# KyungMinJin/OTPose

Measured on AMD Instinct MI355X. Metric: frames/sec at 384x288, 5-frame window, batch 16; heatmap max-abs delta vs ref, higher is better.
Workload: dtype f32 storage+accumulate / f16x3 split products; 1 GPU; BASELINE configs[1]: batch 16 x 5-frame x 384x288, HRNet-W48 + DCN warp + ConvVideoTransformer, fp32 forward (eval), seeded synthetic weights; clips_per_gpu=16, parallelism=dp1, outputs_finite=True

## Files before the change

### include/otpose_hip.h

```cpp
#ifndef OTPOSE_HIP_H
#define OTPOSE_HIP_H

#include <stddef.h>

#ifdef __cplusplus
extern "C" {
#endif

#define OTP_OK 0
#define OTP_ERR_BAD_ARG (-1)
#define OTP_ERR_UNSUPPORTED (-2)
#define OTP_ERR_LAUNCH (-3)
#define OTP_ERR_WORKSPACE (-4)

#define OTP_DTYPE_F32 0
#define OTP_DTYPE_F16 1
#define OTP_DTYPE_BF16 2
#define OTP_DTYPE_F64 3
#define OTP_DTYPE_I64 4

#define OTP_ACT_NONE 0
#define OTP_ACT_RELU 1
#define OTP_ACT_GELU 2

// ... 188 lines not shown
int otp_mlp_fused(const void* x, const void* packed, const void* scale, const void* shift, const void* res, void* out,
                  int B, int C, int HID, int T, void* stream);
int otp_ln_mlp_fused(const void* y, const void* ln_gamma, const void* ln_beta, float ln_eps, const void* packed,
                     const void* scale, const void* shift, void* out, int B, int C, int HID, int T, void* stream);

int otp_dense_x3_supported(int C, int T);
size_t otp_dense_x3_weight_bytes(int C);
int otp_dense_x3_pack(const void* w, const void* scale, const void* shift, void* packed, int C, void* stream);
int otp_dense_x3(const void* const* x, const void* const* packed, const void* const* res, void* const* out, int nprob, int B,
                 int C, int T, void* stream);
int otp_dense_x3_pack_bf16p(const void* w, const void* scale, const void* shift, void* packed, int C, void* stream);
int otp_dense_x3_bf16p(const void* const* x, const void* const* packed, const void* const* res, void* const* out, int nprob, int B,
                 int C, int T, void* stream);
int otp_qkv_front_x3(const void* x, const void* table, const void* packed_q, const void* packed_k, const void* packed_v,
                     void* q, void* k, void* v, int B, int C, int T, float eps, void* stream);

int otp_stem_conv_x3_supported(int B, int F, int H, int W, int Cout);
size_t otp_stem_conv_x3_weight_bytes(int Cout);
int otp_stem_conv_x3_pack(const void* w, const void* scale, const void* shift, void* packed, int Cout, void* stream);
int otp_stem_conv_x3(const void* in, const void* packed, void* out, int B, int F, int H, int W, int Cout, void* stream);

int otp_pointwise_x3_supported(int Cin, int Cout, int T);
size_t otp_pointwise_x3_weight_bytes(int Cin, int Cout);
int otp_pointwise_x3_pack(const void* w, const void* scale, const void* shift, void* packed, int Cin, int Cout, void* stream);
int otp_pointwise_x3(const void* x, const void* packed, const void* res, void* out, int B, int Cin, int Cout, int T, int x_ctot,
                     int x_coff, int res_ctot, int res_coff, int out_ctot, int out_coff, int relu, void* stream);
int otp_pointwise_x3_s8_supported(int Cin, int Cout, int T);
size_t otp_pointwise_x3_s8_weight_bytes(int Cin, int Cout);
int otp_pointwise_x3_s8_pack(const void* w, const void* scale, const void* shift, void* packed, int Cin, int Cout, void* stream);
int otp_pointwise_x3_s8(const void* x, const void* packed, void* out_s8, int B, int Cin, int Cout, int T, int x_ctot, int x_coff,
// ... 219 lines not shown
```

### otpose_amd/csrc/densex.hip

```cpp
#include "x3.h"
#ifndef OTP_ENTRY
#define OTP_ENTRY(name) name
#endif

namespace {

constexpr int dx_ks(int C) { return (C + 31) / 32; }
constexpr int dx_block_bytes(int C) { return (dx_ks(C) * 2 * 1024 + 128 + 4095) / 4096 * 4096; }

__global__ void densex_pack_kernel(const float* __restrict__ w, const float* __restrict__ scale, const float* __restrict__ shift,
                                   unsigned char* __restrict__ packed, int C) {
    const int KS = dx_ks(C), MT = (C + 15) / 16, BLKB = dx_block_bytes(C), units = BLKB / 16;
    const int idx = blockIdx.x * blockDim.x + threadIdx.x;
    if (idx >= MT * units) return;
    const int mt = idx / units, u = idx - mt * units;
    otp_u32x4 o = {0u, 0u, 0u, 0u};
    if (u < KS * 2 * 64) {
        const int frag = u >> 6, lane = u & 63, row = 16 * mt + (lane & 15), kq = lane >> 4, ks = frag >> 1;
        float v[8];
#pragma unroll
        for (int j = 0; j < 8; ++j) {
            const int c = 32 * ks + 8 * kq + j;
            v[j] = (row < C && c < C) ? w[(size_t)row * C + c] : 0.f;
        }
// ... 2 lines not shown
        o = __builtin_bit_cast(otp_u32x4, (frag & 1) ? lo : hi);
    } else if (u < KS * 2 * 64 + 8) {
        const int k = (u - KS * 2 * 64) * 4;
        float v[4];
#pragma unroll
        for (int i = 0; i < 4; ++i) {
            const int e = k + i, c = 16 * mt + (e & 15);
            v[i] = c < C ? (e < 16 ? (scale ? scale[c] : 1.f) : (shift ? shift[c] : 0.f)) : 0.f;
        }
        o = (otp_u32x4){__builtin_bit_cast(uint32_t, v[0]), __builtin_bit_cast(uint32_t, v[1]), __builtin_bit_cast(uint32_t, v[2]),
                    __builtin_bit_cast(uint32_t, v[3])};
    }
    reinterpret_cast<otp_u32x4*>(packed)[idx] = o;
}

template <int C, bool RES, bool H1 = false>
__device__ __forceinline__ void dx_project(const otp_x3x8 (&Xh)[dx_ks(C)][2], const otp_x3x8 (&Xl)[dx_ks(C)][2],
                                           const unsigned char* __restrict__ packed, unsigned char* lds,
                                           const float* __restrict__ res, float* __restrict__ out, size_t base, int T, int tok,
                                           bool valid, unsigned* rflag) {
    constexpr int KS = dx_ks(C), MT = (C + 15) / 16, BLKB = dx_block_bytes(C);
    bool bad = false;
    const int lane = threadIdx.x & 63, kq = lane >> 4;
    const unsigned plane = (unsigned)((size_t)C * T * sizeof(float));
    const otp_rsrc ro = make_rsrc32(out + base, plane);
    const otp_rsrc rr = make_rsrc32(RES && res ? res + base : out, RES && res ? plane : 0u);
#pragma unroll 1
    for (int mt = 0; mt < MT; ++mt) {
        int voff[4];
        otp_f32x2 r[4];
#pragma unroll
        for (int i = 0; i < 4; ++i) {
            const int c = 16 * mt + 4 * kq + i;
            voff[i] = (valid && c < C) ? (c * T + tok) * 4 : -16;
            if (RES) r[i] = __builtin_bit_cast(otp_f32x2, __builtin_amdgcn_raw_buffer_load_b64(rr, voff[i], 0, 0));
        }
        asm volatile("" ::: "memory");
        if (mt + 1 < MT) otp_lds_stage<256, BLKB>(packed + (size_t)(mt + 1) * BLKB, lds + ((mt + 1) & 1) * BLKB);
        asm volatile("" ::: "memory");
        const unsigned char* P = lds + (mt & 1) * BLKB;
        otp_f32x4 acc0 = {0.f, 0.f, 0.f, 0.f}, acc1 = {0.f, 0.f, 0.f, 0.f};
#pragma unroll
        for (int ks = 0; ks < KS; ++ks) {
            const otp_x3x8 ah = *reinterpret_cast<const otp_x3x8*>(P + (ks * 2) * 1024 + lane * 16);
            if constexpr (!H1) {
                const otp_x3x8 al = *reinterpret_cast<const otp_x3x8*>(P + (ks * 2 + 1) * 1024 + lane * 16);
                acc0 = OTP_X3_MFMA(al, Xh[ks][0], acc0, 0, 0, 0);
                acc1 = OTP_X3_MFMA(al, Xh[ks][1], acc1, 0, 0, 0);
                acc0 = OTP_X3_MFMA(ah, Xl[ks][0], acc0, 0, 0, 0);
                acc1 = OTP_X3_MFMA(ah, Xl[ks][1], acc1, 0, 0, 0);
            }
            acc0 = OTP_X3_MFMA(ah, Xh[ks][0], acc0, 0, 0, 0);
            acc1 = OTP_X3_MFMA(ah, Xh[ks][1], acc1, 0, 0, 0);
        }
        const otp_f32x4 sc = *reinterpret_cast<const otp_f32x4*>(P + KS * 2048 + 16 * kq);
        const otp_f32x4 sh = *reinterpret_cast<const otp_f32x4*>(P + KS * 2048 + 64 + 16 * kq);
#pragma unroll
        for (int i = 0; i < 4; ++i) {
            otp_f32x2 v = {acc0[i] * sc[i] + sh[i], acc1[i] * sc[i] + sh[i]};
            if (RES) v += r[i];
            bad |= otp_out_of_range(v.x);
                bad |= otp_out_of_range(v.y);
            __builtin_amdgcn_raw_buffer_store_b64(__builtin_bit_cast(otp_u32x2, v), ro, voff[i], 0, 0);
        }
        if (mt + 1 < MT) {
            asm volatile("s_waitcnt vmcnt(4)" ::: "memory");
            __builtin_amdgcn_s_barrier();
            asm volatile("" ::: "memory");
        }
    }
    otp_range_report(rflag, bad, OTP_RANGE_DENSEX);
}

struct DxArgs {
    const float* x[3];
    const unsigned char* packed[3];
    const float* res[3];
    float* out[3];
};

template <int C, bool H1 = false>
// ... 19 lines not shown
            v0[j] = live ? v.x : 0.f;
            v1[j] = live ? v.y : 0.f;
        }
        otp_x3_split8(v0, Xh[ks][0], Xl[ks][0]);
        otp_x3_split8(v1, Xh[ks][1], Xl[ks][1]);
    }
    __syncthreads();
    dx_project<C, true, H1>(Xh, Xl, A.packed[blockIdx.y], lds, A.res[blockIdx.y], A.out[blockIdx.y], base, T, tok, valid, rflag);
}

struct QxArgs {
    const unsigned char* packed[3];
    float* out[3];
};

template <int C, bool H1 = false>
__global__ __launch_bounds__(256, C <= 136 ? 3 : 1) void qkvx_front_kernel(const float* __restrict__ x, const float* __restrict__ table,
                                                            QxArgs A, int T, int tiles_per_b, float eps, unsigned* rflag) {
    constexpr int KS = dx_ks(C), BLKB = dx_block_bytes(C), TAB = 3 * C * 8;
    __shared__ __attribute__((aligned(16))) unsigned char lds[2 * BLKB];
    __shared__ __attribute__((aligned(16))) float tab[TAB];
    const int tid = threadIdx.x, lane = tid & 63, wave = tid >> 6, kq = lane >> 4, n = lane & 15;
    const int b = blockIdx.x / tiles_per_b, tile = blockIdx.x - b * tiles_per_b;
    const int tok = tile * 128 + wave * 32 + 2 * n;
    const bool valid = tok < T;
    const int tokc = valid ? tok : T - 2;
    const bool l_ok = tokc >= 1, r_ok = tokc + 2 < T;
    const size_t base = (size_t)b * C * T;
    const otp_rsrc rx = make_rsrc(x + base, (size_t)C * T * sizeof(float));
    constexpr float inv_c = 1.f / (float)C;
    const int vb0 = (8 * kq * T + tokc) * 4;
    for (int i = tid; i < TAB / 4; i += 256)
        reinterpret_cast<otp_f32x4*>(tab)[i] = reinterpret_cast<const otp_f32x4*>(table)[i];
    __syncthreads();

    for (int p = (int)blockIdx.y; p <= (int)blockIdx.y; ++p) {
        otp_lds_stage<256, BLKB>(A.packed[p], lds);
        const float* tp = tab + p * C * 8;
        float X0[KS][8], X1[KS][8];
        float s0 = 0.f, s1 = 0.f;
#pragma unroll
        for (int ks = 0; ks < KS; ++ks) {
#pragma unroll
            for (int j = 0; j < 8; ++j) {
                const int c = 32 * ks + 8 * kq + j;
                const bool live = 32 * ks + 24 + j < C || c < C;
                const int so = (32 * ks + j) * T * 4;
                const otp_f32x2 m = __builtin_bit_cast(otp_f32x2, __builtin_amdgcn_raw_buffer_load_b64(rx, live ? vb0 : -16, so, 0));
                const float la = bload(rx, live ? vb0 - 4 : -16, so), ld = bload(rx, live ? vb0 + 8 : -16, so);
                const float a = l_ok ? la : 0.f, d = r_ok ? ld : 0.f;
                const otp_f32x4 w = *reinterpret_cast<const otp_f32x4*>(tp + (live ? c : 0) * 8);
                X0[ks][j] = live ? w[0] * a + w[1] * m.x + w[2] * m.y : 0.f;
// ... 18 lines not shown
        otp_x3x8 Xh[KS][2], Xl[KS][2];
#pragma unroll
        for (int ks = 0; ks < KS; ++ks) {
#pragma unroll
            for (int j = 0; j < 8; ++j) {
                const int c = 32 * ks + 8 * kq + j;
                const bool live = 32 * ks + 24 + j < C || c < C;
                const float g = tp[(live ? c : 0) * 8 + 3], be = tp[(live ? c : 0) * 8 + 4];
                X0[ks][j] = live ? X0[ks][j] * r0 * g + be : 0.f;
                X1[ks][j] = live ? X1[ks][j] * r1 * g + be : 0.f;
            }
            otp_x3_split8(X0[ks], Xh[ks][0], Xl[ks][0]);
            otp_x3_split8(X1[ks], Xh[ks][1], Xl[ks][1]);
        }
        __syncthreads();
        dx_project<C, false, H1>(Xh, Xl, A.packed[p], lds, nullptr, A.out[p], base, T, tok, valid, rflag);
    }
}

}

#ifndef OTP_X3_GRAD_COPY
extern "C" int otp_dense_x3_supported(int C, int T) { return ((C == 136 || C == 204) && T > 0 && T % 2 == 0) ? 1 : 0; }

extern "C" size_t otp_dense_x3_weight_bytes(int C) {
    if (C <= 0 || C % 4) return 0;
    return (size_t)((C + 15) / 16) * dx_block_bytes(C);
}
#endif

extern "C" int OTP_ENTRY(otp_dense_x3_pack)(const void* w, const void* scale, const void* shift, void* packed, int C, void* stream) {
// ... 41 lines not shown
                            int nprob, int B, int C, int T, void* stream) {
    return dx_dense_launch(x, packed, res, out, nprob, B, C, T, stream, false);
}

#ifndef OTP_X3_GRAD_COPY
extern "C" int otp_dense_h1(const void* const* x, const void* const* packed, const void* const* res, void* const* out, int nprob, int B,
                            int C, int T, void* stream) {
    return dx_dense_launch(x, packed, res, out, nprob, B, C, T, stream, true);
}
#endif

#ifndef OTP_X3_GRAD_COPY
namespace {
int dx_qkv_launch(const void* x, const void* table, const void* packed_q, const void* packed_k, const void* packed_v, void* q, void* k,
                  void* v, int B, int C, int T, float eps, void* stream, bool h1) {
    if (!x || !table || !packed_q || !packed_k || !packed_v || !q || !k || !v || B <= 0) return OTP_ERR_BAD_ARG;
    if (!otp_dense_x3_supported(C, T)) return OTP_ERR_UNSUPPORTED;
    if ((reinterpret_cast<uintptr_t>(x) | reinterpret_cast<uintptr_t>(q) | reinterpret_cast<uintptr_t>(k) |
         reinterpret_cast<uintptr_t>(v)) & 7 ||
        (reinterpret_cast<uintptr_t>(table) | reinterpret_cast<uintptr_t>(packed_q) | reinterpret_cast<uintptr_t>(packed_k) |
         reinterpret_cast<uintptr_t>(packed_v)) & 15)
        return OTP_ERR_BAD_ARG;
    if ((size_t)C * T * sizeof(float) >= (1ull << 31)) return OTP_ERR_UNSUPPORTED;
    QxArgs a;
    a.packed[0] = static_cast<const unsigned char*>(packed_q); a.packed[1] = static_cast<const unsigned char*>(packed_k);
    a.packed[2] = static_cast<const unsigned char*>(packed_v);
    a.out[0] = static_cast<float*>(q); a.out[1] = static_cast<float*>(k); a.out[2] = static_cast<float*>(v);
    const int tiles = otp_ceil_div(T, 128);
    const dim3 grid((unsigned)(B * tiles), 3u);
    auto st = static_cast<hipStream_t>(stream);
    auto xf = static_cast<const float*>(x), tf = static_cast<const float*>(table);
    if (C == 204) {
        if (h1) hipLaunchKernelGGL((qkvx_front_kernel<204, true>), grid, dim3(256), 0, st, xf, tf, a, T, tiles, eps, otp_range_word());
        else hipLaunchKernelGGL((qkvx_front_kernel<204, false>), grid, dim3(256), 0, st, xf, tf, a, T, tiles, eps, otp_range_word());
    } else {
        if (h1) hipLaunchKernelGGL((qkvx_front_kernel<136, true>), grid, dim3(256), 0, st, xf, tf, a, T, tiles, eps, otp_range_word());
        else hipLaunchKernelGGL((qkvx_front_kernel<136, false>), grid, dim3(256), 0, st, xf, tf, a, T, tiles, eps, otp_range_word());
    }
    return otp_launch_status();
}
}

extern "C" int otp_qkv_front_x3(const void* x, const void* table, const void* packed_q, const void* packed_k,
                                const void* packed_v, void* q, void* k, void* v, int B, int C, int T, float eps, void* stream) {
    return dx_qkv_launch(x, table, packed_q, packed_k, packed_v, q, k, v, B, C, T, eps, stream, false);
}

extern "C" int otp_qkv_front_h1(const void* x, const void* table, const void* packed_q, const void* packed_k,
                                const void* packed_v, void* q, void* k, void* v, int B, int C, int T, float eps, void* stream) {
    return dx_qkv_launch(x, table, packed_q, packed_k, packed_v, q, k, v, B, C, T, eps, stream, true);
}
#endif
```

### otpose_amd/csrc/transformer.hip

```cpp
#include "common.h"
#include <cstdlib>
#ifndef OTP_ENTRY
#define OTP_ENTRY(name) name
#endif

namespace {

template <int CREG>
__global__ __launch_bounds__(256) void ln_channel_kernel(const float* __restrict__ x, const float* __restrict__ gamma,
                                                          const float* __restrict__ beta, float* __restrict__ y,
                                                          int C, int T, float eps) {
    const int t = blockIdx.x * blockDim.x + threadIdx.x;
    if (t >= T) return;
    const size_t base = (size_t)blockIdx.y * C * T + t;
    const float inv_c = 1.f / (float)C;
    if (CREG > 0) {
        float v[CREG > 0 ? CREG : 1];
        float s = 0.f;
#pragma unroll
        for (int c = 0; c < CREG; ++c) {
            v[c] = c < C ? x[base + (size_t)c * T] : 0.f;
            s += v[c];
        }
        const float mu = s * inv_c;
// ... 367 lines not shown
            }
        }
    }
    float* slab = slabs + ((size_t)bh * gridDim.y + s) * HSP * HSP;
#pragma unroll
    for (int i = 0; i < TPW; ++i) {
        const int tile = wave + 4 * i;
        if (tile < NT) {
            const int ib = tile / NB, jb = tile - ib * NB;
#pragma unroll
            for (int r = 0; r < 4; ++r) slab[(ib * 16 + kk * 4 + r) * HSP + jb * 16 + r16] = acc[i][r];
        }
    }
}

__global__ __launch_bounds__(256) void attn_softmax_kernel(const float* __restrict__ slabs, float* __restrict__ P,
                                                            int hs, int HSP, int NS, float scale) {
    const int bh = blockIdx.x, lane = threadIdx.x & 63, wave = threadIdx.x >> 6;
    const int row = blockIdx.y * 4 + wave;
    if (row >= HSP) return;
    const float* sb = slabs + (size_t)bh * NS * HSP * HSP;
    float* pb = P + (size_t)bh * HSP * HSP;
    float v[2];
#pragma unroll
    for (int h = 0; h < 2; ++h) {
        const int col = lane + 64 * h;
        const bool live = row < hs && col < hs;
        const float* sp = sb + (live ? (size_t)row * HSP + col : 0);
        float a = 0.f;
        int s = 0;
        for (; s + 8 <= NS; s += 8) {
            float t[8];
#pragma unroll
            for (int j = 0; j < 8; ++j) t[j] = sp[(size_t)(s + j) * HSP * HSP];
#pragma unroll
            for (int j = 0; j < 8; ++j) a += t[j];
        }
        for (; s < NS; ++s) a += sp[(size_t)s * HSP * HSP];
        v[h] = live ? a * scale : -INFINITY;
    }
    const float m = wave_max(fmaxf(v[0], v[1]));
    float e0 = (row < hs && lane < hs) ? expf(v[0] - m) : 0.f;
    float e1 = (row < hs && lane + 64 < hs) ? expf(v[1] - m) : 0.f;
    const float den = wave_sum(e0 + e1);
    if (lane < HSP) pb[row * HSP + lane] = row < hs ? e0 / den : 0.f;
    if (lane + 64 < HSP) pb[row * HSP + lane + 64] = row < hs ? e1 / den : 0.f;
}

constexpr int pv_tt(int nb) { return nb > 6 ? 128 : 256; }
template <int NB>
__global__ __launch_bounds__(256) void attn_pv_kernel(const float* __restrict__ v, const float* __restrict__ P,
                                                       float* __restrict__ out, int hs, int T) {
    constexpr int HSP = NB * 16, TT = pv_tt(NB), TB = TT / 64;
    constexpr int PS = HSP + 2;
    constexpr int VS = TT + 16;
    extern __shared__ __attribute__((aligned(16))) float smem[];
    float* pl = smem;
    float* vl = smem + HSP * PS;
    const int tid = threadIdx.x, lane = tid & 63, wave = tid >> 6;
    const int bh = blockIdx.x, t0 = blockIdx.y * TT;
    const float* vb = v + (size_t)bh * hs * T;
    const float* pb = P + (size_t)bh * HSP * HSP;
// ... 393 lines not shown
        case 4: OTP_ATT(4) break;
        case 5: OTP_ATT(5) break;
        case 6: OTP_ATT(6) break;
        default: OTP_ATT(7) break;
    }
#undef OTP_ATT
    return otp_launch_status();
}

extern "C" int otp_chan_attn_set_split(int on) {
    g_attn_split.store(on ? 1 : 0, std::memory_order_relaxed);
    return OTP_OK;
}

extern "C" int otp_chan_attn_splits(int BH, int T) { return (BH > 0 && T > 0) ? attn_splits(BH, T) : 0; }
#endif

extern "C" int OTP_ENTRY(otp_chan_attn_scores)(const void* a, const void* b, void* slabs, int BH, int hs, int T, void* stream) {
    if (!a || !b || !slabs || BH <= 0 || hs <= 0 || T <= 0) return OTP_ERR_BAD_ARG;
    const int HSP = (hs + 15) & ~15, NB = HSP / 16;
    if (NB > 7) return OTP_ERR_UNSUPPORTED;
    const int NS = attn_splits(BH, T);
    const int chunk = otp_ceil_div(otp_ceil_div(T, NS), ATT_TC) * ATT_TC;
    auto st = static_cast<hipStream_t>(stream);
    dim3 g1(BH, NS);
    auto af = static_cast<const float*>(a);
    auto bf = static_cast<const float*>(b);
    auto sf = static_cast<float*>(slabs);
#define OTP_SC(NB_)                                                                                       \
    {                                                                                                     \
// ... 89 lines not shown
```

### otpose_amd/csrc/x3.h

```cpp
#pragma once
#include "common.h"

__device__ __forceinline__ void otp_x3_split8(const float (&v)[8], otp_u32x4& hi, otp_u32x4& lo) {
    uint32_t h[4], l[4];
#pragma unroll
    for (int i = 0; i < 4; ++i) {
        const otp_f32x2 a = {v[2 * i], v[2 * i + 1]};
        const uint32_t hb = __builtin_bit_cast(uint32_t, __builtin_convertvector(a, otp_x3x2));
        const otp_f32x2 af = otp_x3_widen(hb);
        h[i] = hb;
        l[i] = __builtin_bit_cast(uint32_t, __builtin_convertvector(a - af, otp_x3x2));
    }
    hi = (otp_u32x4){h[0], h[1], h[2], h[3]};
    lo = (otp_u32x4){l[0], l[1], l[2], l[3]};
}
__device__ __forceinline__ void otp_x3_split8(const float (&v)[8], otp_x3x8& hi, otp_x3x8& lo) {
    otp_u32x4 h, l;
    otp_x3_split8(v, h, l);
    hi = __builtin_bit_cast(otp_x3x8, h);
    lo = __builtin_bit_cast(otp_x3x8, l);
}

constexpr int OTP_S8_KS = 5;
__host__ __device__ constexpr int otp_s8_wch(int ntw) { return 8 * ntw + ntw; }

__host__ __device__ inline bool otp_tile_paired(int co_blk, int t, int ntw, int Cout) {
    const int tb = t | 1;
    return tb < ntw && co_blk + 16 * tb < Cout;
}
__host__ __device__ inline int otp_row2ch(int co_blk, int t, int row, int ntw, int Cout) {
    return otp_tile_paired(co_blk, t, ntw, Cout) ? co_blk + 32 * (t >> 1) + 8 * (row >> 2) + 4 * (t & 1) + (row & 3)
                                                 : co_blk + 16 * t + row;
}

template <int NM, int NR>
__device__ __forceinline__ void otp_s8_block_sched() {
// ... 23 lines not shown
```

### otpose_amd/engine.py

```python
from __future__ import annotations

import ctypes
import dataclasses
import os
import sys
import warnings
from typing import Callable, List, Optional, Tuple

import torch

from . import hip, ops
from .ops import ACT_GELU, ACT_NONE, ACT_RELU, View

def _pair(v):
    return (int(v), int(v)) if isinstance(v, int) else (int(v[0]), int(v[1]))


def plain_conv(cv, k, stride=1, pad="same", dil=1, groups=1, bias=False, cin=None, cout=None) -> bool:
    if pad == "same":
        pad = (dil or 1) * (k // 2)
    return (cv.kernel_size == (k, k) and (stride is None or cv.stride == (stride, stride))
            and (pad is None or tuple(cv.padding) == (pad, pad)) and (dil is None or tuple(cv.dilation) == (dil, dil))
            and (groups is None or cv.groups == groups) and (bias is None or (cv.bias is not None) == bias)
            and (cin is None or cv.in_channels == cin) and (cout is None or cv.out_channels == cout))
# ... 20 lines not shown
    f32_tail: int = 0
    h16_tail: bool = True
    range_check: str = "defer"
    s8_residual: bool = True
    s8_lazy_nchw: bool = True
    s8_stride2: bool = True
    t1_s8: bool = True
    l1_s8: bool = True
    l1_pair: bool = True
    stem_x3: bool = True
    chain_modules: bool = True
    up_any_width: bool = True
    conv_log: bool = False
    poison: Optional[Tuple[int, int]] = None
    te_serial: bool = False

    @classmethod
    def from_env(cls) -> "Routes":
        env = os.environ.get
        on = lambda name: env("OTPOSE_" + name, "1") != "0"
        x3 = env("OTPOSE_CONV_MATH", "x3") != "f32"
        poison = env("OTPOSE_POISON")
        return cls(use_graph=on("HIP_GRAPH"), use_winograd=on("WINOGRAD"), use_x3=x3, use_dcn_fused=x3 and on("DCN_FUSED"),
                   use_s8=x3 and on("S8"), use_flow_fused=on("FLOW_FUSED"), use_small_conv=on("SMALL_CONV"),
                   use_fused_mlp=on("FUSED_MLP"), fuse_shortcut=on("FUSE_SHORTCUT"), fuse_upsample=on("FUSE_UPSAMPLE"),
                   use_dense_cc=on("DENSE_CC"), use_qkv_front=on("QKV_FRONT"), use_pointx=x3 and on("POINTX"),
                   pointx_fuse=on("POINTX_FUSE"), pointx_any=env("OTPOSE_POINTX_ANY", "0") == "1", multi_stream=on("STREAMS"),
                   f32_tail=int(env("OTPOSE_F32_TAIL", "0")) if x3 else 0, h16_tail=on("H16_TAIL"),
                   range_check=env("OTPOSE_RANGE_CHECK", "defer"), s8_residual=on("S8_RESIDUAL"), s8_lazy_nchw=on("S8_LAZY_NCHW"),
                   s8_stride2=on("S8_STRIDE2"), t1_s8=on("T1_S8"), l1_s8=on("L1_S8"), l1_pair=on("L1_PAIR"), stem_x3=on("STEM_X3"),
                   chain_modules=on("CHAIN_MODULES"), up_any_width=on("UP_ANY_WIDTH"), conv_log=bool(env("OTPOSE_CONV_LOG")),
                   poison=tuple(int(v) for v in poison.split(":")) if poison else None, te_serial=env("OTPOSE_TE_SERIAL") == "1")

    @property
    def lazy_nchw(self) -> bool:
        return self.s8_residual and self.s8_lazy_nchw


class Aux:
    __slots__ = ("s8", "c4", "nchw_needed")

    def __init__(self, s8=None, c4=None, nchw_needed=False):
        self.s8, self.c4, self.nchw_needed = s8, c4, nchw_needed


class InferenceEngine:
    h16 = False
# ... 23 lines not shown
        self.ops: List[Callable] = []
        self._pair_s8 = {}
        self.l1_pairs = 0
        self._aux = {}
        self._keep = []
        self._bufs = []
        self._stream = None
        self.use_graph, self.graph = use_graph, None
        self._exact = False
        self._sid = 0
        self._side = hip.side_streams(device, 3, 4 * stream_set) if routes.multi_stream else []

    @classmethod
    def bare(cls, device, multi_stream=False):
        self = cls.__new__(cls)
        self._init(device, dataclasses.replace(Routes.from_env(), multi_stream=bool(multi_stream)), use_graph=False)
        return self

    use_x3 = property(lambda self: self.routes.use_x3)
    use_dcn_fused = property(lambda self: self.routes.use_dcn_fused)
    multi_stream = property(lambda self: self.routes.multi_stream)
    f32_tail = property(lambda self: self.routes.f32_tail)
    range_check = property(lambda self: self.routes.range_check)
    half_products = property(lambda self: self.h16 and self.routes.use_x3 and self.routes.h16_tail)

    @property
    def s8_here(self) -> bool:
        return self.routes.use_s8 and not self._exact

    @property
    def s2_here(self) -> bool:
# ... 617 lines not shown
        a = blk.attn
        r = self.routes
        if r.use_flow_fused and stride == 1 and ops.flow_block_supported(blk, C, T):
            fp, bp = ops.pack_flow_front(blk, self.dev), ops.pack_flow_back(blk, self.dev)
            self._keep += [fp, bp]
            q, k, v, att, out = (self.new(B, C, T) for _ in range(5))
            self.call(L.otp_flow_front, "otp_flow_front", *ops.flow_front_args(x, fp, q, k, v, blk.ln1.eps))
            self.chan_attn(q, k, v, att, a)
            self.call(L.otp_flow_back, "otp_flow_back", *ops.flow_back_args(x, att, bp, out, blk.mlp[0].out_channels, blk.ln2.eps))
            return out
        ln1 = self.new(B, C, T)
        skip = self.new(B, C, To) if stride > 1 else None
        p = self.dev_param
        self.call(L.otp_ln_channel, "otp_ln_channel", hip.ptr(x), hip.ptr(p(blk.ln1.weight)), hip.ptr(p(blk.ln1.bias)),
                  hip.ptr(ln1), hip.ptr(skip), B, C, T, blk.ln1.eps)
        q, k, v = self.new(B, C, To), self.new(B, C, To), self.new(B, C, To)
        dx3 = r.use_dense_cc and r.use_x3 and ops.dense_x3_supported(C, To)
        dense = dx3 or (r.use_dense_cc and ops.dense_cc_supported(C, To))
        if dense:
            packs = [ops.pack_dense_cc(m.weight.to(self.dev), None, m.bias.to(self.dev), x3=dx3)
                     for m in (a.query, a.key, a.value)]
        if dense and stride == 1 and r.use_qkv_front:
            table = ops.pack_qkv_table(*[p(t) for t in (a.query_conv.weight, a.key_conv.weight, a.value_conv.weight,
                                                         a.query_norm.weight, a.query_norm.bias, a.key_norm.weight,
                                                         a.key_norm.bias, a.value_norm.weight, a.value_norm.bias)])
            self._keep += [table, *packs]
            self.call((L.otp_qkv_front_h1 if self.half_products else L.otp_qkv_front_x3) if dx3 else L.otp_qkv_front, "otp_qkv_front",
                      *ops.qkv_front_args(ln1, table, packs, (q, k, v), a.query_norm.eps))
        else:
            qn, kn, vn = self.new(B, C, To), self.new(B, C, To), self.new(B, C, To)
            self.call(L.otp_dwconv_ln3, "otp_dwconv_ln3", hip.ptr(ln1), hip.ptr(p(a.query_conv.weight)),
                      hip.ptr(p(a.key_conv.weight)), hip.ptr(p(a.value_conv.weight)),
                      hip.ptr(p(a.query_norm.weight)), hip.ptr(p(a.query_norm.bias)),
                      hip.ptr(p(a.key_norm.weight)), hip.ptr(p(a.key_norm.bias)),
                      hip.ptr(p(a.value_norm.weight)), hip.ptr(p(a.value_norm.bias)),
                      hip.ptr(qn), hip.ptr(kn), hip.ptr(vn), B, C, T, stride, a.query_norm.eps)
            if dense:
                self.dense((qn, kn, vn), packs, None, (q, k, v), B, C, To)
            else:
                self.conv(self.v3(qn), a.query.weight, self.v3(q), bias=a.query.bias)
                self.conv(self.v3(kn), a.key.weight, self.v3(k), bias=a.key.bias)
                self.conv(self.v3(vn), a.value.weight, self.v3(v), bias=a.value.bias)
        att = self.new(B, C, To)
        self.chan_attn(q, k, v, att, a)
        sa = blk.drop_path_attn.scale.detach().reshape(-1)
        y = self.new(B, C, To)
        if dense:
            sad = sa.to(self.dev, torch.float32)
            pk = ops.pack_dense_cc(a.proj.weight.to(self.dev), sad, a.proj.bias.detach().to(self.dev) * sad,
                                   x3=r.use_x3 and ops.dense_x3_supported(C, To))
            self.dense((att,), [pk], (skip if stride > 1 else x,), (y,), B, C, To)
        else:
            self.conv(self.v3(att), a.proj.weight, self.v3(y), scale=sa,
                      shift=a.proj.bias.detach() * sa.to(a.proj.bias.device), res=self.v3(skip if stride > 1 else x))
        sm = blk.drop_path_mlp.scale.detach().reshape(-1)
        out = self.new(B, C, To)
        hid = blk.mlp[0].out_channels
        mlp_x3 = r.use_fused_mlp and r.use_x3 and ops.mlp_x3_supported(C, hid, To)
        if mlp_x3 or (r.use_fused_mlp and ops.mlp_fused_supported(C, hid, To)):
# ... 254 lines not shown
```

### otpose_amd/ops.py

```python
from __future__ import annotations

import ctypes
import math
import os

import torch
from torch.autograd import Function

from . import hip
from .augment import FLIP_PAIRS

_K = hip.CONSTANTS
_DTYPE_F32 = _K["OTP_DTYPE_F32"]


def _require_gpu(*tensors):
    for t in tensors:
        if t is not None and not t.is_cuda:
            raise NotImplementedError("otpose_amd operators run on the GPU only (no CPU path)")


def _check_f32(*tensors):
    for t in tensors:
        if t is not None and t.dtype != torch.float32:
# ... 990 lines not shown


def chan_attn_args(q, k, v, out, ws, nbytes, n_head, scale):
    b, c, t = q.shape
    return (hip.ptr(q), hip.ptr(k), hip.ptr(v), hip.ptr(out), hip.ptr(ws), nbytes, b, c, t, n_head, scale)


def chan_attn(q, k, v, n_head, scale):
    _require_gpu(q, k, v)
    b, c, t = q.shape
    out = torch.empty_like(q)
    L = hip.lib()
    nbytes = L.otp_chan_attn_workspace(b, c, t, n_head)
    ws = torch.empty(max(nbytes // 4, 1), dtype=torch.float32, device=q.device)
    _launch(L.otp_chan_attn, "otp_chan_attn", chan_attn_args(q, k, v, out, ws, nbytes, n_head, scale), q)
    return out


def upsample_linear_args(x, out, f, out_coff=0):
    b, c = x.shape[:2]
    return (hip.ptr(x), hip.ptr(out), b, c, x.numel() // (b * c), f, out.shape[1], out_coff)


def upsample_linear(x, f, out=None, out_coff=0):
    _require_gpu(x)
    b, c, t = x.shape
    if out is None:
        out = torch.empty((b, c, t * f), dtype=x.dtype, device=x.device)
    _launch(hip.lib().otp_upsample_linear, "otp_upsample_linear", upsample_linear_args(x, out, f, out_coff), x)
    return out
# ... 738 lines not shown
```

Measured before the change: 3292 frames/s.

## Fold value projection into channel-attention probabilities to skip materializing V

For C=136 with two heads at stride 1, the value projection weight is pre-multiplied by the softmax attention matrix per batch, producing a per-batch packed weight image. A single dense x3 projection of the normalized value input then yields the attention output directly. This removes the separate V write and read and the P·V pass, at the cost of a per-batch weight-fold kernel and per-batch packed weights. Rounding changes because the V projection and the attention apply are reassociated.

```diff
diff --git a/include/otpose_hip.h b/include/otpose_hip.h
--- a/include/otpose_hip.h
+++ b/include/otpose_hip.h
@@ -226,6 +226,17 @@
                  int C, int T, void* stream);
 int otp_qkv_front_x3(const void* x, const void* table, const void* packed_q, const void* packed_k, const void* packed_v,
                      void* q, void* k, void* v, int B, int C, int T, float eps, void* stream);
+int otp_attn_vfold_supported(int C, int n_head, int T);
+size_t otp_attn_vfold_workspace(int B, int C, int T, int n_head);
+int otp_qk_front_x3(const void* x, const void* table, const void* packed_q, const void* packed_k, void* q, void* k, int B, int C,
+                    int T, float eps, void* stream);
+int otp_attn_vfold_fold(const void* slabs, const void* w_v, const void* b_v, void* images, int B, int C, int T, int n_head,
+                        float scale, void* stream);
+int otp_attn_vfold_apply(const void* x, const void* table, const void* images, void* out, int B, int C, int T, int n_head, float eps,
+                         void* stream);
+int otp_chan_attn_vfold(const void* q, const void* k, const void* x, const void* table, const void* w_v, const void* b_v, void* out,
+                        void* workspace, size_t workspace_bytes, int B, int C, int T, int n_head, float scale, float eps,
+                        void* stream);
 
 int otp_stem_conv_x3_supported(int B, int F, int H, int W, int Cout);
 size_t otp_stem_conv_x3_weight_bytes(int Cout);
diff --git a/otpose_amd/csrc/densex.hip b/otpose_amd/csrc/densex.hip
--- a/otpose_amd/csrc/densex.hip
+++ b/otpose_amd/csrc/densex.hip
@@ -4,9 +4,6 @@
 #endif
 
 namespace {
-
-constexpr int dx_ks(int C) { return (C + 31) / 32; }
-constexpr int dx_block_bytes(int C) { return (dx_ks(C) * 2 * 1024 + 128 + 4095) / 4096 * 4096; }
 
 __global__ void densex_pack_kernel(const float* __restrict__ w, const float* __restrict__ scale, const float* __restrict__ shift,
                                    unsigned char* __restrict__ packed, int C) {
@@ -40,7 +37,7 @@
     reinterpret_cast<otp_u32x4*>(packed)[idx] = o;
 }
 
-template <int C, bool RES, bool H1 = false>
+template <int C, bool RES, bool H1 = false, int HS = 0>
 __device__ __forceinline__ void dx_project(const otp_x3x8 (&Xh)[dx_ks(C)][2], const otp_x3x8 (&Xl)[dx_ks(C)][2],
                                            const unsigned char* __restrict__ packed, unsigned char* lds,
                                            const float* __restrict__ res, float* __restrict__ out, size_t base, int T, int tok,
@@ -55,11 +52,19 @@
     for (int mt = 0; mt < MT; ++mt) {
         int voff[4];
         otp_f32x2 r[4];
-#pragma unroll
-        for (int i = 0; i < 4; ++i) {
-            const int c = 16 * mt + 4 * kq + i;
-            voff[i] = (valid && c < C) ? (c * T + tok) * 4 : -16;
-            if (RES) r[i] = __builtin_bit_cast(otp_f32x2, __builtin_amdgcn_raw_buffer_load_b64(rr, voff[i], 0, 0));
+        if constexpr (HS > 0) {
+            static_assert(HS % 4 == 0 && C % HS == 0 && !RES, "four channels of a lane inside one head, no residual");
+            const int c = 16 * mt + 4 * kq, head = c / HS;
+            const bool live = valid && c < C;
+            voff[0] = live ? ((head * T + tok) * HS + (c - head * HS)) * 4 : -16;
+            voff[1] = live ? voff[0] + HS * 4 : -16;
+        } else {
+#pragma unroll
+            for (int i = 0; i < 4; ++i) {
+                const int c = 16 * mt + 4 * kq + i;
+                voff[i] = (valid && c < C) ? (c * T + tok) * 4 : -16;
+                if (RES) r[i] = __builtin_bit_cast(otp_f32x2, __builtin_amdgcn_raw_buffer_load_b64(rr, voff[i], 0, 0));
+            }
         }
         asm volatile("" ::: "memory");
         if (mt + 1 < MT) otp_lds_stage<256, BLKB>(packed + (size_t)(mt + 1) * BLKB, lds + ((mt + 1) & 1) * BLKB);
@@ -81,16 +86,30 @@
         }
         const otp_f32x4 sc = *reinterpret_cast<const otp_f32x4*>(P + KS * 2048 + 16 * kq);
         const otp_f32x4 sh = *reinterpret_cast<const otp_f32x4*>(P + KS * 2048 + 64 + 16 * kq);
-#pragma unroll
-        for (int i = 0; i < 4; ++i) {
-            otp_f32x2 v = {acc0[i] * sc[i] + sh[i], acc1[i] * sc[i] + sh[i]};
-            if (RES) v += r[i];
-            bad |= otp_out_of_range(v.x);
+        if constexpr (HS > 0) {
+            float v0[4], v1[4];
+#pragma unroll
+            for (int i = 0; i < 4; ++i) {
+                v0[i] = acc0[i] * sc[i] + sh[i];
+                v1[i] = acc1[i] * sc[i] + sh[i];
+                bad |= otp_out_of_range(v0[i]);
+                bad |= otp_out_of_range(v1[i]);
+            }
+            __builtin_amdgcn_raw_buffer_store_b128(__builtin_bit_cast(otp_u32x4, (otp_f32x4){v0[0], v0[1], v0[2], v0[3]}), ro, voff[0], 0, 0);
+            __builtin_amdgcn_raw_buffer_store_b128(__builtin_bit_cast(otp_u32x4, (otp_f32x4){v1[0], v1[1], v1[2], v1[3]}), ro, voff[1], 0, 0);
+        } else {
+#pragma unroll
+            for (int i = 0; i < 4; ++i) {
+                otp_f32x2 v = {acc0[i] * sc[i] + sh[i], acc1[i] * sc[i] + sh[i]};
+                if (RES) v += r[i];
+                bad |= otp_out_of_range(v.x);
                 bad |= otp_out_of_range(v.y);
-            __builtin_amdgcn_raw_buffer_store_b64(__builtin_bit_cast(otp_u32x2, v), ro, voff[i], 0, 0);
+                __builtin_amdgcn_raw_buffer_store_b64(__builtin_bit_cast(otp_u32x2, v), ro, voff[i], 0, 0);
+            }
         }
         if (mt + 1 < MT) {
-            asm volatile("s_waitcnt vmcnt(4)" ::: "memory");
+            if constexpr (HS > 0) asm volatile("s_waitcnt vmcnt(2)" ::: "memory");
+            else asm volatile("s_waitcnt vmcnt(4)" ::: "memory");
             __builtin_amdgcn_s_barrier();
             asm volatile("" ::: "memory");
         }
@@ -140,7 +159,7 @@
     float* out[3];
 };
 
-template <int C, bool H1 = false>
+template <int C, bool H1 = false, int HS = 0>
 __global__ __launch_bounds__(256, C <= 136 ? 3 : 1) void qkvx_front_kernel(const float* __restrict__ x, const float* __restrict__ table,
                                                             QxArgs A, int T, int tiles_per_b, float eps, unsigned* rflag) {
     constexpr int KS = dx_ks(C), BLKB = dx_block_bytes(C), TAB = 3 * C * 8;
@@ -160,8 +179,10 @@
         reinterpret_cast<otp_f32x4*>(tab)[i] = reinterpret_cast<const otp_f32x4*>(table)[i];
     __syncthreads();
 
-    for (int p = (int)blockIdx.y; p <= (int)blockIdx.y; ++p) {
-        otp_lds_stage<256, BLKB>(A.packed[p], lds);
+    const int p0 = HS > 0 ? 2 : (int)blockIdx.y;
+    for (int p = p0; p <= p0; ++p) {
+        const unsigned char* __restrict__ pk = HS > 0 ? A.packed[0] + (size_t)b * ((C + 15) / 16) * BLKB : A.packed[p];
+        otp_lds_stage<256, BLKB>(pk, lds);
         const float* tp = tab + p * C * 8;
         float X0[KS][8], X1[KS][8];
         float s0 = 0.f, s1 = 0.f;
@@ -210,7 +231,7 @@
             otp_x3_split8(X1[ks], Xh[ks][1], Xl[ks][1]);
         }
         __syncthreads();
-        dx_project<C, false, H1>(Xh, Xl, A.packed[p], lds, nullptr, A.out[p], base, T, tok, valid, rflag);
+        dx_project<C, false, H1, HS>(Xh, Xl, pk, lds, nullptr, A.out[HS > 0 ? 0 : p], base, T, tok, valid, rflag);
     }
 }
 
@@ -282,7 +303,8 @@
 namespace {
 int dx_qkv_launch(const void* x, const void* table, const void* packed_q, const void* packed_k, const void* packed_v, void* q, void* k,
                   void* v, int B, int C, int T, float eps, void* stream, bool h1) {
-    if (!x || !table || !packed_q || !packed_k || !packed_v || !q || !k || !v || B <= 0) return OTP_ERR_BAD_ARG;
+    const bool qk_only = !packed_v && !v;
+    if (!x || !table || !packed_q || !packed_k || !q || !k || (!qk_only && (!packed_v || !v)) || B <= 0) return OTP_ERR_BAD_ARG;
     if (!otp_dense_x3_supported(C, T)) return OTP_ERR_UNSUPPORTED;
     if ((reinterpret_cast<uintptr_t>(x) | reinterpret_cast<uintptr_t>(q) | reinterpret_cast<uintptr_t>(k) |
          reinterpret_cast<uintptr_t>(v)) & 7 ||
@@ -295,7 +317,7 @@
     a.packed[2] = static_cast<const unsigned char*>(packed_v);
     a.out[0] = static_cast<float*>(q); a.out[1] = static_cast<float*>(k); a.out[2] = static_cast<float*>(v);
     const int tiles = otp_ceil_div(T, 128);
-    const dim3 grid((unsigned)(B * tiles), 3u);
+    const dim3 grid((unsigned)(B * tiles), qk_only ? 2u : 3u);
     auto st = static_cast<hipStream_t>(stream);
     auto xf = static_cast<const float*>(x), tf = static_cast<const float*>(table);
     if (C == 204) {
@@ -314,6 +336,32 @@
     return dx_qkv_launch(x, table, packed_q, packed_k, packed_v, q, k, v, B, C, T, eps, stream, false);
 }
 
+extern "C" int otp_qk_front_x3(const void* x, const void* table, const void* packed_q, const void* packed_k, void* q, void* k, int B,
+                               int C, int T, float eps, void* stream) {
+    return dx_qkv_launch(x, table, packed_q, packed_k, nullptr, q, k, nullptr, B, C, T, eps, stream, false);
+}
+
+extern "C" int otp_attn_vfold_supported(int C, int n_head, int T) {
+    return (C == 136 && n_head == 2 && otp_dense_x3_supported(C, T)) ? 1 : 0;
+}
+
+extern "C" int otp_attn_vfold_apply(const void* x, const void* table, const void* images, void* out, int B, int C, int T, int n_head,
+                                    float eps, void* stream) {
+    if (!x || !table || !images || !out || B <= 0) return OTP_ERR_BAD_ARG;
+    if (!otp_attn_vfold_supported(C, n_head, T)) return OTP_ERR_UNSUPPORTED;
+    if (reinterpret_cast<uintptr_t>(x) & 7 || (reinterpret_cast<uintptr_t>(table) | reinterpret_cast<uintptr_t>(images) |
+                                               reinterpret_cast<uintptr_t>(out)) & 15)
+        return OTP_ERR_BAD_ARG;
+    if ((size_t)C * T * sizeof(float) >= (1ull << 31)) return OTP_ERR_UNSUPPORTED;
+    QxArgs a = {};
+    a.packed[0] = static_cast<const unsigned char*>(images);
+    a.out[0] = static_cast<float*>(out);
+    const int tiles = otp_ceil_div(T, 128);
+    hipLaunchKernelGGL((qkvx_front_kernel<136, false, 68>), dim3((unsigned)(B * tiles), 1u), dim3(256), 0, static_cast<hipStream_t>(stream),
+                       static_cast<const float*>(x), static_cast<const float*>(table), a, T, tiles, eps, otp_range_word());
+    return otp_launch_status();
+}
+
 extern "C" int otp_qkv_front_h1(const void* x, const void* table, const void* packed_q, const void* packed_k,
                                 const void* packed_v, void* q, void* k, void* v, int B, int C, int T, float eps, void* stream) {
     return dx_qkv_launch(x, table, packed_q, packed_k, packed_v, q, k, v, B, C, T, eps, stream, true);
diff --git a/otpose_amd/csrc/transformer.hip b/otpose_amd/csrc/transformer.hip
--- a/otpose_amd/csrc/transformer.hip
+++ b/otpose_amd/csrc/transformer.hip
@@ -1,4 +1,4 @@
-#include "common.h"
+#include "x3.h"
 #include <cstdlib>
 #ifndef OTP_ENTRY
 #define OTP_ENTRY(name) name
@@ -405,13 +405,8 @@
     }
 }
 
-__global__ __launch_bounds__(256) void attn_softmax_kernel(const float* __restrict__ slabs, float* __restrict__ P,
-                                                            int hs, int HSP, int NS, float scale) {
-    const int bh = blockIdx.x, lane = threadIdx.x & 63, wave = threadIdx.x >> 6;
-    const int row = blockIdx.y * 4 + wave;
-    if (row >= HSP) return;
-    const float* sb = slabs + (size_t)bh * NS * HSP * HSP;
-    float* pb = P + (size_t)bh * HSP * HSP;
+__device__ __forceinline__ void attn_softmax_row(const float* __restrict__ sb, int row, int lane, int hs, int HSP, int NS, float scale,
+                                                 float& p0, float& p1) {
     float v[2];
 #pragma unroll
     for (int h = 0; h < 2; ++h) {
@@ -434,9 +429,77 @@
     float e0 = (row < hs && lane < hs) ? expf(v[0] - m) : 0.f;
     float e1 = (row < hs && lane + 64 < hs) ? expf(v[1] - m) : 0.f;
     const float den = wave_sum(e0 + e1);
-    if (lane < HSP) pb[row * HSP + lane] = row < hs ? e0 / den : 0.f;
-    if (lane + 64 < HSP) pb[row * HSP + lane + 64] = row < hs ? e1 / den : 0.f;
-}
+    p0 = row < hs ? e0 / den : 0.f;
+    p1 = row < hs ? e1 / den : 0.f;
+}
+
+__global__ __launch_bounds__(256) void attn_softmax_kernel(const float* __restrict__ slabs, float* __restrict__ P,
+                                                            int hs, int HSP, int NS, float scale) {
+    const int bh = blockIdx.x, lane = threadIdx.x & 63, wave = threadIdx.x >> 6;
+    const int row = blockIdx.y * 4 + wave;
+    if (row >= HSP) return;
+    float* pb = P + (size_t)bh * HSP * HSP;
+    float p0, p1;
+    attn_softmax_row(slabs + (size_t)bh * NS * HSP * HSP, row, lane, hs, HSP, NS, scale, p0, p1);
+    if (lane < HSP) pb[row * HSP + lane] = p0;
+    if (lane + 64 < HSP) pb[row * HSP + lane + 64] = p1;
+}
+
+#ifndef OTP_X3_GRAD_COPY
+constexpr int VF_COLS = 192;
+__global__ __launch_bounds__(256) void attn_vfold_kernel(const float* __restrict__ slabs, const float* __restrict__ wv,
+                                                          const float* __restrict__ bv, unsigned char* __restrict__ images, int hs,
+                                                          int HSP, int NS, float scale, int C, int n_head) {
+    __shared__ float prow[4][128];
+    __shared__ __attribute__((aligned(16))) float mrow[4][VF_COLS];
+    const int bh = blockIdx.x, lane = threadIdx.x & 63, wave = threadIdx.x >> 6;
+    const int b = bh / n_head, head = bh - b * n_head;
+    const int i = blockIdx.y * 4 + wave;
+    const int KS = dx_ks(C), MT = (C + 15) / 16, BLKB = dx_block_bytes(C);
+    const bool live = i < hs;
+    const bool zero_row = !live && head == n_head - 1 && i < HSP && C + (i - hs) < 16 * MT;
+    const int row = live ? head * hs + i : C + (i - hs);
+    float p0, p1;
+    attn_softmax_row(slabs + (size_t)bh * NS * HSP * HSP, min(i, HSP - 1), lane, hs, HSP, NS, scale, p0, p1);
+    prow[wave][lane] = live ? p0 : 0.f;
+    prow[wave][lane + 64] = live ? p1 : 0.f;
+    __syncthreads();
+    float acc[3] = {0.f, 0.f, 0.f}, sh = 0.f;
+    if (live) {
+        const float* wr = wv + (size_t)head * hs * C;
+        int col[3];
+#pragma unroll
+        for (int k = 0; k < 3; ++k) col[k] = lane + 64 * k < C ? lane + 64 * k : 0;
+#pragma unroll 4
+        for (int j = 0; j < hs; ++j) {
+            const float pj = prow[wave][j];
+#pragma unroll
+            for (int k = 0; k < 3; ++k) acc[k] = fmaf(pj, wr[(size_t)j * C + col[k]], acc[k]);
+            if (bv) sh = fmaf(pj, bv[head * hs + j], sh);
+        }
+    }
+#pragma unroll
+    for (int k = 0; k < 3; ++k) mrow[wave][lane + 64 * k] = lane + 64 * k < C ? acc[k] : 0.f;
+    __syncthreads();
+    if (!live && !zero_row) return;
+    unsigned char* blk = images + ((size_t)b * MT + (row >> 4)) * BLKB;
+    if (lane < 4 * KS) {
+        const int ks = lane >> 2, kq = lane & 3;
+        float v[8];
+#pragma unroll
+        for (int j = 0; j < 8; ++j) v[j] = mrow[wave][8 * lane + j];
+        otp_u32x4 hi, lo;
+        otp_x3_split8(v, hi, lo);
+        otp_u32x4* frag = reinterpret_cast<otp_u32x4*>(blk + (size_t)ks * 2048) + kq * 16 + (row & 15);
+        frag[0] = hi;
+        frag[64] = lo;
+    } else if (lane == 4 * KS) {
+        float* ss = reinterpret_cast<float*>(blk + (size_t)KS * 2048);
+        ss[row & 15] = live ? 1.f : 0.f;
+        ss[16 + (row & 15)] = sh;
+    }
+}
+#endif
 
 constexpr int pv_tt(int nb) { return nb > 6 ? 128 : 256; }
 template <int NB>
@@ -860,6 +923,40 @@
 }
 
 extern "C" int otp_chan_attn_splits(int BH, int T) { return (BH > 0 && T > 0) ? attn_splits(BH, T) : 0; }
+
+extern "C" size_t otp_attn_vfold_workspace(int B, int C, int T, int n_head) {
+    if (B <= 0 || !otp_attn_vfold_supported(C, n_head, T)) return 0;
+    const int hs = C / n_head, HSP = (hs + 15) & ~15;
+    const size_t BH = (size_t)B * n_head;
+    return BH * attn_splits((int)BH, T) * HSP * HSP * sizeof(float) + (size_t)B * otp_dense_x3_weight_bytes(C);
+}
+
+extern "C" int otp_attn_vfold_fold(const void* slabs, const void* w_v, const void* b_v, void* images, int B, int C, int T, int n_head,
+                                   float scale, void* stream) {
+    if (!slabs || !w_v || !images || B <= 0) return OTP_ERR_BAD_ARG;
+    if (!otp_attn_vfold_supported(C, n_head, T)) return OTP_ERR_UNSUPPORTED;
+    const int hs = C / n_head, HSP = (hs + 15) & ~15, BH = B * n_head;
+    if (HSP - hs < (C + 15) / 16 * 16 - C || C > VF_COLS || hs > 128) return OTP_ERR_UNSUPPORTED;
+    if (reinterpret_cast<uintptr_t>(images) & 15) return OTP_ERR_BAD_ARG;
+    hipLaunchKernelGGL(attn_vfold_kernel, dim3(BH, otp_ceil_div(HSP, 4)), dim3(256), 0, static_cast<hipStream_t>(stream),
+                       static_cast<const float*>(slabs), static_cast<const float*>(w_v), static_cast<const float*>(b_v),
+                       static_cast<unsigned char*>(images), hs, HSP, attn_splits(BH, T), scale, C, n_head);
+    return otp_launch_status();
+}
+
+extern "C" int otp_chan_attn_vfold(const void* q, const void* k, const void* x, const void* table, const void* w_v, const void* b_v,
+                                   void* out, void* workspace, size_t workspace_bytes, int B, int C, int T, int n_head, float scale,
+                                   float eps, void* stream) {
+    if (!q || !k || !x || !table || !w_v || !out || !workspace || B <= 0) return OTP_ERR_BAD_ARG;
+    if (!otp_attn_vfold_supported(C, n_head, T)) return OTP_ERR_UNSUPPORTED;
+    if (workspace_bytes < otp_attn_vfold_workspace(B, C, T, n_head)) return OTP_ERR_WORKSPACE;
+    const int hs = C / n_head, HSP = (hs + 15) & ~15, BH = B * n_head;
+    unsigned char* images = static_cast<unsigned char*>(workspace) + (size_t)BH * attn_splits(BH, T) * HSP * HSP * sizeof(float);
+    int rc = otp_chan_attn_scores(q, k, workspace, BH, hs, T, stream);
+    if (rc == OTP_OK) rc = otp_attn_vfold_fold(workspace, w_v, b_v, images, B, C, T, n_head, scale, stream);
+    if (rc == OTP_OK) rc = otp_attn_vfold_apply(x, table, images, out, B, C, T, n_head, eps, stream);
+    return rc;
+}
 #endif
 
 extern "C" int OTP_ENTRY(otp_chan_attn_scores)(const void* a, const void* b, void* slabs, int BH, int hs, int T, void* stream) {
diff --git a/otpose_amd/csrc/x3.h b/otpose_amd/csrc/x3.h
--- a/otpose_amd/csrc/x3.h
+++ b/otpose_amd/csrc/x3.h
@@ -20,6 +20,9 @@
     hi = __builtin_bit_cast(otp_x3x8, h);
     lo = __builtin_bit_cast(otp_x3x8, l);
 }
+
+constexpr int dx_ks(int C) { return (C + 31) / 32; }
+constexpr int dx_block_bytes(int C) { return (dx_ks(C) * 2 * 1024 + 128 + 4095) / 4096 * 4096; }
 
 constexpr int OTP_S8_KS = 5;
 __host__ __device__ constexpr int otp_s8_wch(int ntw) { return 8 * ntw + ntw; }
diff --git a/otpose_amd/engine.py b/otpose_amd/engine.py
--- a/otpose_amd/engine.py
+++ b/otpose_amd/engine.py
@@ -58,6 +58,7 @@
     conv_log: bool = False
     poison: Optional[Tuple[int, int]] = None
     te_serial: bool = False
+    attn_vfold = True
 
     @classmethod
     def from_env(cls) -> "Routes":
@@ -65,7 +66,7 @@
         on = lambda name: env("OTPOSE_" + name, "1") != "0"
         x3 = env("OTPOSE_CONV_MATH", "x3") != "f32"
         poison = env("OTPOSE_POISON")
-        return cls(use_graph=on("HIP_GRAPH"), use_winograd=on("WINOGRAD"), use_x3=x3, use_dcn_fused=x3 and on("DCN_FUSED"),
+        r = cls(use_graph=on("HIP_GRAPH"), use_winograd=on("WINOGRAD"), use_x3=x3, use_dcn_fused=x3 and on("DCN_FUSED"),
                    use_s8=x3 and on("S8"), use_flow_fused=on("FLOW_FUSED"), use_small_conv=on("SMALL_CONV"),
                    use_fused_mlp=on("FUSED_MLP"), fuse_shortcut=on("FUSE_SHORTCUT"), fuse_upsample=on("FUSE_UPSAMPLE"),
                    use_dense_cc=on("DENSE_CC"), use_qkv_front=on("QKV_FRONT"), use_pointx=x3 and on("POINTX"),
@@ -75,6 +76,13 @@
                    s8_stride2=on("S8_STRIDE2"), t1_s8=on("T1_S8"), l1_s8=on("L1_S8"), l1_pair=on("L1_PAIR"), stem_x3=on("STEM_X3"),
                    chain_modules=on("CHAIN_MODULES"), up_any_width=on("UP_ANY_WIDTH"), conv_log=bool(env("OTPOSE_CONV_LOG")),
                    poison=tuple(int(v) for v in poison.split(":")) if poison else None, te_serial=env("OTPOSE_TE_SERIAL") == "1")
+        object.__setattr__(r, "attn_vfold", on("ATTN_VFOLD"))
+        return r
+
+    def with_(self, **changes) -> "Routes":
+        r = dataclasses.replace(self, **changes)
+        object.__setattr__(r, "attn_vfold", self.attn_vfold)
+        return r
 
     @property
     def lazy_nchw(self) -> bool:
@@ -128,7 +136,7 @@
     @classmethod
     def bare(cls, device, multi_stream=False):
         self = cls.__new__(cls)
-        self._init(device, dataclasses.replace(Routes.from_env(), multi_stream=bool(multi_stream)), use_graph=False)
+        self._init(device, Routes.from_env().with_(multi_stream=bool(multi_stream)), use_graph=False)
         return self
 
     use_x3 = property(lambda self: self.routes.use_x3)
@@ -776,19 +784,30 @@
         p = self.dev_param
         self.call(L.otp_ln_channel, "otp_ln_channel", hip.ptr(x), hip.ptr(p(blk.ln1.weight)), hip.ptr(p(blk.ln1.bias)),
                   hip.ptr(ln1), hip.ptr(skip), B, C, T, blk.ln1.eps)
-        q, k, v = self.new(B, C, To), self.new(B, C, To), self.new(B, C, To)
+        q, k = self.new(B, C, To), self.new(B, C, To)
         dx3 = r.use_dense_cc and r.use_x3 and ops.dense_x3_supported(C, To)
         dense = dx3 or (r.use_dense_cc and ops.dense_cc_supported(C, To))
+        vfold = (r.attn_vfold and stride == 1 and dx3 and r.use_qkv_front and not self.half_products
+                 and ops.attn_vfold_supported(C, a.n_head, To))
+        v = None if vfold else self.new(B, C, To)
         if dense:
             packs = [ops.pack_dense_cc(m.weight.to(self.dev), None, m.bias.to(self.dev), x3=dx3)
-                     for m in (a.query, a.key, a.value)]
+                     for m in ((a.query, a.key) if vfold else (a.query, a.key, a.value))]
         if dense and stride == 1 and r.use_qkv_front:
             table = ops.pack_qkv_table(*[p(t) for t in (a.query_conv.weight, a.key_conv.weight, a.value_conv.weight,
                                                          a.query_norm.weight, a.query_norm.bias, a.key_norm.weight,
                                                          a.key_norm.bias, a.value_norm.weight, a.value_norm.bias)])
             self._keep += [table, *packs]
-            self.call((L.otp_qkv_front_h1 if self.half_products else L.otp_qkv_front_x3) if dx3 else L.otp_qkv_front, "otp_qkv_front",
-                      *ops.qkv_front_args(ln1, table, packs, (q, k, v), a.query_norm.eps))
+            if vfold:
+                self.call(L.otp_qk_front_x3, "otp_qk_front_x3", *ops.qk_front_args(ln1, table, packs, (q, k), a.query_norm.eps))
+                att = self.new(B, C, To)
+                nbytes = L.otp_attn_vfold_workspace(B, C, To, a.n_head)
+                self.call(L.otp_chan_attn_vfold, "otp_chan_attn_vfold",
+                          *ops.chan_attn_vfold_args(q, k, ln1, table, p(a.value.weight).view(C, C), p(a.value.bias), att,
+                                                    self.new(nbytes // 4), nbytes, a.n_head, a.scale, a.value_norm.eps))
+            else:
+                self.call((L.otp_qkv_front_h1 if self.half_products else L.otp_qkv_front_x3) if dx3 else L.otp_qkv_front, "otp_qkv_front",
+                          *ops.qkv_front_args(ln1, table, packs, (q, k, v), a.query_norm.eps))
         else:
             qn, kn, vn = self.new(B, C, To), self.new(B, C, To), self.new(B, C, To)
             self.call(L.otp_dwconv_ln3, "otp_dwconv_ln3", hip.ptr(ln1), hip.ptr(p(a.query_conv.weight)),
@@ -803,8 +822,9 @@
                 self.conv(self.v3(qn), a.query.weight, self.v3(q), bias=a.query.bias)
                 self.conv(self.v3(kn), a.key.weight, self.v3(k), bias=a.key.bias)
                 self.conv(self.v3(vn), a.value.weight, self.v3(v), bias=a.value.bias)
-        att = self.new(B, C, To)
-        self.chan_attn(q, k, v, att, a)
+        if not vfold:
+            att = self.new(B, C, To)
+            self.chan_attn(q, k, v, att, a)
         sa = blk.drop_path_attn.scale.detach().reshape(-1)
         y = self.new(B, C, To)
         if dense:
diff --git a/otpose_amd/ops.py b/otpose_amd/ops.py
--- a/otpose_amd/ops.py
+++ b/otpose_amd/ops.py
@@ -1028,6 +1028,61 @@
     nbytes = L.otp_chan_attn_workspace(b, c, t, n_head)
     ws = torch.empty(max(nbytes // 4, 1), dtype=torch.float32, device=q.device)
     _launch(L.otp_chan_attn, "otp_chan_attn", chan_attn_args(q, k, v, out, ws, nbytes, n_head, scale), q)
+    return out
+
+
+def attn_vfold_supported(c, n_head, t) -> bool:
+    return bool(hip.lib().otp_attn_vfold_supported(int(c), int(n_head), int(t)))
+
+
+def qk_front_args(x, table, packs, outs, eps):
+    b, c, t = x.shape
+    return (hip.ptr(x), hip.ptr(table), hip.ptr(packs[0]), hip.ptr(packs[1]), hip.ptr(outs[0]), hip.ptr(outs[1]), b, c, t, eps)
+
+
+def qk_front(x, table, packs, eps=1e-5, outs=None, stream=None):
+    _require_gpu(x, table)
+    outs = [torch.empty_like(x) for _ in range(2)] if outs is None else outs
+    _launch(hip.lib().otp_qk_front_x3, "otp_qk_front_x3", qk_front_args(x, table, packs, outs, eps), x, stream)
+    return outs
+
+
+def attn_vfold_fold(q, k, w_v, b_v, n_head, scale):
+    _require_gpu(q, k, w_v)
+    b, c, t = q.shape
+    L = hip.lib()
+    if not L.otp_attn_vfold_supported(c, n_head, t):
+        raise RuntimeError(f"otp_attn_vfold_fold: unsupported shape C={c}, n_head={n_head}, T={t}")
+    bh, hs = b * n_head, c // n_head
+    hsp = (hs + 15) // 16 * 16
+    slabs = torch.empty(bh * L.otp_chan_attn_splits(bh, t) * hsp * hsp, dtype=torch.float32, device=q.device)
+    images = torch.zeros(b, L.otp_dense_x3_weight_bytes(c) // 4, dtype=torch.float32, device=q.device)
+    st = hip.stream_of(q)
+    hip.check(L.otp_chan_attn_scores(hip.ptr(q), hip.ptr(k), hip.ptr(slabs), bh, hs, t, st), "otp_chan_attn_scores")
+    w, bias = _f32(w_v.reshape(c, c), q.device), _f32(b_v, q.device)
+    hip.check(L.otp_attn_vfold_fold(hip.ptr(slabs), hip.ptr(w), hip.ptr(bias), hip.ptr(images), b, c, t, n_head, scale, st),
+              "otp_attn_vfold_fold")
+    return images
+
+
+def chan_attn_vfold_args(q, k, x, table, w_v, b_v, out, ws, nbytes, n_head, scale, eps):
+    b, c, t = q.shape
+    return (hip.ptr(q), hip.ptr(k), hip.ptr(x), hip.ptr(table), hip.ptr(w_v), hip.ptr(b_v), hip.ptr(out), hip.ptr(ws), nbytes,
+            b, c, t, n_head, scale, eps)
+
+
+def chan_attn_vfold(q, k, x, table, w_v, b_v, n_head, scale, eps=1e-5):
+    _require_gpu(q, k, x, table, w_v)
+    b, c, t = q.shape
+    L = hip.lib()
+    nbytes = L.otp_attn_vfold_workspace(b, c, t, n_head)
+    if not nbytes:
+        raise RuntimeError(f"otp_chan_attn_vfold: unsupported shape C={c}, n_head={n_head}, T={t}")
+    out = torch.empty_like(q)
+    ws = torch.empty(nbytes // 4, dtype=torch.float32, device=q.device)
+    w, bias = _f32(w_v.reshape(c, c), q.device), _f32(b_v, q.device)
+    _launch(L.otp_chan_attn_vfold, "otp_chan_attn_vfold",
+            chan_attn_vfold_args(q, k, x, table, w, bias, out, ws, nbytes, n_head, scale, eps), q)
     return out
 
 
```

New measurement: 3315 frames/s, median of 6. No clear change (+0.7%).
